# tqch/v-diffusion-torch

Hardware: AMD Instinct MI355X
Metric: train_images_per_sec (higher is better)
Workload: dtype fp32 (bf16x3 split products in the tile-engine GEMMs)

## Files before the change

### v-diffusion-torch_amd/csrc/gemm.hip

```cpp
#include "common.h"
#include <math.h>
#include <stdlib.h>
#include <type_traits>

namespace {

constexpr int KT = 32;
#ifndef VD_GEMM_SPLIT_DEFAULT
#define VD_GEMM_SPLIT_DEFAULT 1
#endif

struct GemmArgs {
    const float* A; const float* B; float* C; const float* bias; const float* R;
    int M, N, K;
    long long lda, ldb, ldc, ldr;
    int nh;
    long long sAb, sAh, sBb, sBh, sCb, sCh, sRb, sRh;
    float alpha; int accumulate;
    int H, W, Cin;
    int kt_total, kt_per_split;
    long long slab_stride;
    float* colsum; int colsum_accumulate;
    int probe;
    float* stats; int stats_hw;
// ... 283 lines not shown
                o[0] = st1; o[p.N] = st2;
            }
        }
    }
}


typedef __attribute__((address_space(3))) void* lds_ptr_t;
constexpr unsigned OOB = 0x80000000u;
#ifndef VD_SCHED_INTERLEAVE
#define VD_SCHED_INTERLEAVE 1
#endif

__device__ __forceinline__ __amdgpu_buffer_rsrc_t make_rsrc(const float* base, int records = (int)OOB) {
    return __builtin_amdgcn_make_buffer_rsrc((void*)base, 0, records, 0x00020000);
}


__device__ __forceinline__ void pix_yx(const GemmArgs& p, int pix, int& y, int& x) {
    if (p.lgW >= 0) { const int rem = pix & ((1 << p.lgHW) - 1); y = rem >> p.lgW; x = rem & ((1 << p.lgW) - 1); }
    else { const int rem = pix % (p.H * p.W); y = rem / p.W; x = rem % p.W; }
}
template <int KT>
__device__ __forceinline__ int swz_of(int row) { return KT == 32 ? ((row >> 1) & 7) : ((row >> 2) & 3); }
template <int KT>
__device__ __forceinline__ int row_swz_t(int row, int chunk) { return row * KT + ((chunk ^ swz_of<KT>(row)) << 2); }

constexpr int VD_GROUP_MAX = 36;
struct GroupPtrs { const float* A[VD_GROUP_MAX]; const float* B[VD_GROUP_MAX]; };
struct NoGroup {};
struct GroupOut { float* C[VD_GROUP_MAX]; float* cs[VD_GROUP_MAX]; };

typedef __bf16 bf16x8 __attribute__((ext_vector_type(8)));
typedef __bf16 bf16x2 __attribute__((ext_vector_type(2)));
__device__ __forceinline__ unsigned pk_bf16(float a, float b) {
    const bf16x2 v = {(__bf16)a, (__bf16)b};
    return __builtin_bit_cast(unsigned, v);
}
__device__ __forceinline__ void split8(const float (&x)[8], bf16x8& H, bf16x8& M, bf16x8& L) {
    typedef unsigned u32x4 __attribute__((ext_vector_type(4)));
    u32x4 h, m, l;
#pragma unroll
    for (int q = 0; q < 4; ++q) {
        const float x0 = x[2 * q], x1 = x[2 * q + 1];
        const unsigned hp = pk_bf16(x0, x1);
        const float r0 = x0 - __uint_as_float(hp << 16), r1 = x1 - __uint_as_float(hp & 0xFFFF0000u);
        const unsigned mp = pk_bf16(r0, r1);
        const float s0 = r0 - __uint_as_float(mp << 16), s1 = r1 - __uint_as_float(mp & 0xFFFF0000u);
        h[q] = hp; m[q] = mp; l[q] = pk_bf16(s0, s1);
    }
    H = __builtin_bit_cast(bf16x8, h); M = __builtin_bit_cast(bf16x8, m); L = __builtin_bit_cast(bf16x8, l);
}

#ifndef VD_KT16_BLOCKS
#define VD_KT16_BLOCKS 4
#endif
#ifndef VD_SPL_BLOCKS
#define VD_SPL_BLOCKS 2
#endif
template <int BM, int BN, int AK, int BK, bool SPLITK, int KT, bool TR, bool GROUPED, bool SPL>
__device__ __forceinline__ void gemm_dma_body(const GemmArgs& p, const std::conditional_t<GROUPED, GroupPtrs, NoGroup>& gp) {
    constexpr int NBUF = 2;
    __shared__ __attribute__((aligned(1024))) float smem[NBUF * (BM + BN) * KT];
    constexpr int MT = BM / 64, NT = BN / 64;
    constexpr int AIT = BM * KT / 1024, BIT = BN * KT / 1024;
    constexpr int A_LPR = BM / 4, B_LPR = BN / 4;
    constexpr int A_RPP = 64 / A_LPR, B_RPP = 64 / B_LPR;
    constexpr int RLPR = KT / 4, RRPP = 64 / RLPR;
    constexpr bool A2 = (AK == VD_COL) && (MT == 2);
    constexpr bool B2 = (BK != VD_ROW) && (NT == 2);
    typedef float f32x2 __attribute__((ext_vector_type(2)));

    const int tid = threadIdx.x, lane = tid & 63;
    const int wave = __builtin_amdgcn_readfirstlane(tid >> 6);
    const int li = lane & 31, lh = lane >> 5;
    const int wm = (wave >> 1) * (BM / 2), wn = (wave & 1) * (BN / 2);
    int tbx = blockIdx.x, tby = blockIdx.y, tbz = blockIdx.z;
    {
        const unsigned T = gridDim.x * gridDim.y * gridDim.z;
        const unsigned lin = (blockIdx.z * gridDim.y + blockIdx.y) * gridDim.x + blockIdx.x;
        if (T >= 16) {
            const unsigned q = T / 8, r = T % 8, xcd = lin % 8, slot = lin / 8;
            const unsigned t = (xcd < r ? xcd * (q + 1) : r * (q + 1) + (xcd - r) * q) + slot;
            tbx = t % gridDim.x; tby = (t / gridDim.x) % gridDim.y; tbz = t / (gridDim.x * gridDim.y);
        }
    }
    const int m0 = tby * BM;
    int n0 = tbx * BN;
    int tapN = 0, ci0 = 0;
    if (BK == VD_IM2COL) {
        const int cchN = (p.Cin + BN - 1) / BN;
        tapN = tbx / cchN;
        ci0 = (tbx % cchN) * BN;
        n0 = tapN * p.Cin + ci0;
    }
    const float* A = p.A;
    const float* B = p.B;
    float* C = p.C;
    const float* R = p.R;
    const float* biasp = p.bias;
    int kt_begin = 0, kt_end = p.kt_total;
    if (SPLITK) {
        int slab = tbz;
        if constexpr (GROUPED) {
            const int e = tbz / p.group_S;
            slab = tbz - e * p.group_S;
            A = gp.A[e];
            B = gp.B[e];
        }
        kt_begin = slab * p.kt_per_split;
        kt_end = min(kt_begin + p.kt_per_split, p.kt_total);
        C += (long long)tbz * p.slab_stride;
    } else {
        const int zb = tbz / p.nh, zh = tbz % p.nh;
        A += zb * p.sAb + zh * p.sAh;
        B += zb * p.sBb + zh * p.sBh;
        C += zb * p.sCb + zh * p.sCh;
        if (R) R += zb * p.sRb + zh * p.sRh;
        if (biasp) biasp += zb * p.sBias;
    }

    unsigned voA[AIT], voB[BIT];
    unsigned mkA[AIT];
    int kcA[AIT], kcB[BIT];
    int by[BIT], bx[BIT];
    int tapA = (AK == VD_IM2COL) ? kt_begin % 9 : 0, ccA = (AK == VD_IM2COL) ? kt_begin / 9 : 0;
    const int kinc_x = (BK == VD_IM2COL) ? KT % p.W : 0, kinc_y = (BK == VD_IM2COL) ? KT / p.W : 0;
#pragma unroll
    for (int j = 0; j < AIT; ++j) {
        const int q = j * 4 + wave;
        if (AK == VD_COL) {
            const int kk = q * A_RPP + lane / A_LPR, cm = (lane % A_LPR) * 4;
            const int rowoff = (GROUPED && p.a_kblk) ? (kk >> 4) * (int)p.a_kblk + (kk & 15) * (int)p.lda : kk * (int)p.lda;
            voA[j] = (m0 + cm < p.M) ? (unsigned)(rowoff + cm) * 4u : OOB;
            kcA[j] = kk; mkA[j] = 0;
        } else {
            const int row = q * RRPP + lane / RLPR;
            const int c = (lane % RLPR) ^ swz_of<KT>(row);
            const int m = m0 + row;
// ... 433 lines not shown
                    if (R) t = __builtin_bit_cast(float, __builtin_amdgcn_raw_buffer_load_b32(rrs, (int)vor, rs * ldr4, 0));
                    if (p.accumulate) t += __builtin_bit_cast(float, __builtin_amdgcn_raw_buffer_load_b32(crs, (int)voc, rs * ldc4, 0));
                }
                addv[r] = t;
            }
#pragma unroll
            for (int r = 0; r < 16; r += 2) {
                const int rs0 = A2 ? 2 * ((r & 3) + 8 * (r >> 2)) + a : 32 * a + (r & 3) + 8 * (r >> 2);
                const int rs1 = A2 ? rs0 + 2 : rs0 + 1;
                f32x2 v = {acc[a][b][r], acc[a][b][r + 1]};
                if (!SPLITK) {
                    const f32x2 al = {p.alpha, p.alpha}, bb = {bv, bv}, ad = {addv[r], addv[r + 1]};
                    v = (v * al + bb) + ad;
                    if (want_stats) {
                        if (!edge) { st1p += v; st2p += v * v; }
                        else {
                            if (rs0 + row_lane < rows_valid) { st1 += v[0]; st2 += v[0] * v[0]; }
                            if (rs1 + row_lane < rows_valid) { st1 += v[1]; st2 += v[1] * v[1]; }
                        }
                    }
                }
                const float v0 = v[0], v1 = v[1];
                __builtin_amdgcn_raw_buffer_store_b32(__float_as_uint(v0), crs, (int)voc, rs0 * ldc4, 0);
                __builtin_amdgcn_raw_buffer_store_b32(__float_as_uint(v1), crs, (int)voc, rs1 * ldc4, 0);
            }
        }
        st1 += st1p[0] + st1p[1];
        st2 += st2p[0] + st2p[1];
        if (want_stats && nok) {
            st1 += __shfl_xor(st1, 32, 64);
            st2 += __shfl_xor(st2, 32, 64);
            const int mrow = m0 + wm;
            if (lh == 0 && mrow < p.M) {
                const int chunks = p.stats_hw / (BM / 2);
                float* o = p.stats + ((long long)(mrow / p.stats_hw) * chunks + (mrow % p.stats_hw) / (BM / 2)) * 2 * p.N + n;
                o[0] = st1; o[p.N] = st2;
            }
        }
    }
    stamp_end();
}

template <int BM, int BN, int AK, int BK, bool SPLITK, int KT, bool TR, bool GROUPED = false>
__global__ __launch_bounds__(256, (KT == 16 ? VD_KT16_BLOCKS : 2)) void gemm_dma_kernel(const GemmArgs p,
                                                                                          const std::conditional_t<GROUPED, GroupPtrs, NoGroup> gp) {
    gemm_dma_body<BM, BN, AK, BK, SPLITK, KT, TR, GROUPED, false>(p, gp);
}
template <int BM, int BN, int AK, int BK, bool SPLITK, int KT, bool TR, bool GROUPED = false>
__global__ __launch_bounds__(256, (KT == 16 ? VD_SPL_BLOCKS : 2)) void gemm_split_kernel(const GemmArgs p,
                                                                                           const std::conditional_t<GROUPED, GroupPtrs, NoGroup> gp) {
    gemm_dma_body<BM, BN, AK, BK, SPLITK, KT, TR, GROUPED, true>(p, gp);
}

__global__ __launch_bounds__(512) void wgrad_planes256_kernel(const GemmArgs p, const GroupPtrs gp) {
    constexpr int BM = 256, BN = 256, KTT = 16, NBUF = 3, STG = (BM + BN) * KTT;
    __shared__ __attribute__((aligned(1024))) float smem[NBUF * STG];
    typedef float f32x2 __attribute__((ext_vector_type(2)));
    const int tid = threadIdx.x, lane = tid & 63;
    const int wave = __builtin_amdgcn_readfirstlane(tid >> 6);
    const int li = lane & 31, lh = lane >> 5;
    const int wm = (wave >> 1) * 64, wn = (wave & 1) * 128;
    const int tbx = blockIdx.x, tby = blockIdx.y, tbz = blockIdx.z;
    const int m0 = tby * BM, n0 = tbx * BN;
    const int e = tbz / p.group_S, slab = tbz - e * p.group_S;
    const float* A = gp.A[e] + m0;
    const float* B = gp.B[e] + n0;
    const int kt_begin = slab * p.kt_per_split, kt_end = min(kt_begin + p.kt_per_split, p.kt_total);
    float* C = p.C + (long long)tbz * p.slab_stride;

    auto issue = [&](int kt, int buf) {
        float* as = smem + buf * STG;
        float* bs = as + BM * KTT;
        const int rec = kt < kt_end ? (int)OOB : 0;
        const __amdgpu_buffer_rsrc_t rsA = make_rsrc(A + (p.a_kblk ? (long long)kt * p.a_kblk : (long long)kt * KTT * p.lda), rec);
        const __amdgpu_buffer_rsrc_t rsB = make_rsrc(B + (p.b_kblk ? (long long)kt * p.b_kblk : (long long)kt * KTT * p.ldb), rec);
#pragma unroll
        for (int h = 0; h < 2; ++h) {
            const int kk = wave + 8 * h;
            __builtin_amdgcn_raw_ptr_buffer_load_lds(rsA, (lds_ptr_t)(as + kk * BM), 16, lane * 16, kk * (int)p.lda * 4, 0, 0);
            __builtin_amdgcn_raw_ptr_buffer_load_lds(rsB, (lds_ptr_t)(bs + kk * BN), 16, lane * 16, kk * (int)p.ldb * 4, 0, 0);
        }
    };

    f32x16 acc[2][4];
#pragma unroll
    for (int a = 0; a < 2; ++a)
#pragma unroll
        for (int b = 0; b < 4; ++b)
#pragma unroll
            for (int r = 0; r < 16; ++r) acc[a][b][r] = 0.f;
    float csum[2] = {0.f, 0.f};
    const bool do_cs = p.colsum != nullptr && tbx == 0 && (wave & 1) == 0;

    if (kt_begin < kt_end) {
        issue(kt_begin, 0);
        issue(kt_begin + 1, 1);
        asm volatile("s_waitcnt vmcnt(4)" ::: "memory");
        asm volatile("s_waitcnt lgkmcnt(0)\n\ts_barrier" ::: "memory");
        int buf = 0;
        for (int kt = kt_begin; kt < kt_end; ++kt) {
            const float* as = smem + buf * STG;
            const float* bs = as + BM * KTT;
            issue(kt + 2, buf >= 1 ? buf - 1 : 2);
            float fa[2][8];
            f32x4 fbq[8];
#pragma unroll
            for (int j = 0; j < 8; ++j) {
                const f32x2 v = *reinterpret_cast<const f32x2*>(as + (8 * lh + j) * BM + wm + 2 * li);
                fa[0][j] = v[0]; fa[1][j] = v[1];
                fbq[j] = *reinterpret_cast<const f32x4*>(bs + (8 * lh + j) * BN + wn + 4 * li);
            }
            bf16x8 ah[2], am[2], al[2];
#pragma unroll
            for (int a = 0; a < 2; ++a) split8(fa[a], ah[a], am[a], al[a]);
            if (do_cs) {
                asm volatile("" ::: "memory");
#pragma unroll
                for (int a = 0; a < 2; ++a)
                    csum[a] += ((fa[a][0] + fa[a][1]) + (fa[a][2] + fa[a][3])) + ((fa[a][4] + fa[a][5]) + (fa[a][6] + fa[a][7]));
            }
#pragma unroll
            for (int hb = 0; hb < 2; ++hb) {
                bf16x8 bh[2], bm[2], bl[2];
#pragma unroll
                for (int b2 = 0; b2 < 2; ++b2) {
                    float fb[8];
#pragma unroll
                    for (int j = 0; j < 8; ++j) fb[j] = fbq[j][2 * hb + b2];
                    split8(fb, bh[b2], bm[b2], bl[b2]);
                }
#pragma unroll
                for (int a = 0; a < 2; ++a)
#pragma unroll
                    for (int b2 = 0; b2 < 2; ++b2) {
                        f32x16& d = acc[a][2 * hb + b2];
                        d = __builtin_amdgcn_mfma_f32_32x32x16_bf16(bl[b2], ah[a], d, 0, 0, 0);
                        d = __builtin_amdgcn_mfma_f32_32x32x16_bf16(bh[b2], al[a], d, 0, 0, 0);
                        d = __builtin_amdgcn_mfma_f32_32x32x16_bf16(bm[b2], am[a], d, 0, 0, 0);
                        d = __builtin_amdgcn_mfma_f32_32x32x16_bf16(bh[b2], am[a], d, 0, 0, 0);
                        d = __builtin_amdgcn_mfma_f32_32x32x16_bf16(bm[b2], ah[a], d, 0, 0, 0);
                        d = __builtin_amdgcn_mfma_f32_32x32x16_bf16(bh[b2], ah[a], d, 0, 0, 0);
                    }
            }
            asm volatile("s_waitcnt vmcnt(4)" ::: "memory");
            asm volatile("s_waitcnt lgkmcnt(0)\n\ts_barrier" ::: "memory");
            buf = buf == 2 ? 0 : buf + 1;
        }
    }
    asm volatile("s_waitcnt vmcnt(0)" ::: "memory");

    if (do_cs) {
#pragma unroll
        for (int a = 0; a < 2; ++a) {
            const float v = csum[a] + __shfl_xor(csum[a], 32, 64);
            if (lh == 0) p.colsum[(long long)tbz * p.M + m0 + wm + 2 * li + a] = v;
        }
    }
    typedef unsigned u32x4 __attribute__((ext_vector_type(4)));
    const __amdgpu_buffer_rsrc_t crs = make_rsrc(C + (long long)m0 * p.N + n0);
#pragma unroll
    for (int a = 0; a < 2; ++a) {
        const unsigned rowb = (unsigned)(wm + 2 * li + a) * (unsigned)p.N * 4u;
#pragma unroll
        for (int r = 0; r < 16; ++r) {
            const int i = (r & 3) + 8 * (r >> 2) + 4 * lh;
            const u32x4 u = {__float_as_uint(acc[a][0][r]), __float_as_uint(acc[a][1][r]), __float_as_uint(acc[a][2][r]), __float_as_uint(acc[a][3][r])};
            __builtin_amdgcn_raw_buffer_store_b128(u, crs, (int)(rowb + (unsigned)(wn + 4 * i) * 4u), 0, 0);
        }
    }
}

__global__ void reduce_slabs_kernel(const float* slabs, int S, long long slab_stride, int M, int N, float* out,
                                    long long ldo, int accumulate, float alpha, const float* cpart, float* colsum,
                                    int colsum_accumulate) {
    const long long idx = (long long)blockIdx.x * blockDim.x + threadIdx.x;
    if (colsum && idx < M) {
        float c = 0.f;
        for (int z = 0; z < S; ++z) c += cpart[(long long)z * M + idx];
        colsum[idx] = colsum_accumulate ? colsum[idx] + c : c;
    }
    if (idx >= (long long)M * N) return;
    float s = 0.f;
    for (int z = 0; z < S; ++z) s += slabs[z * slab_stride + idx];
    const int m = idx / N, n = idx % N;
    float* o = out + (long long)m * ldo + n;
    s *= alpha;
    *o = accumulate ? *o + s : s;
}

__global__ void reduce_slabs_grouped_kernel(const float* slabs, int S, long long slab_stride, int M, int N, const GroupOut outs,
                                            long long ldo, const float* cpart) {
    const int e = blockIdx.y;
    const long long idx = (long long)blockIdx.x * blockDim.x + threadIdx.x;
    const float* sl = slabs + (long long)e * S * slab_stride;
    float* cs = outs.cs[e];
    if (cs && idx < M) {
        float c = 0.f;
        for (int z = 0; z < S; ++z) c += cpart[((long long)e * S + z) * M + idx];
        cs[idx] = c;
    }
    if (idx >= (long long)M * N) return;
    float s = 0.f;
    for (int z = 0; z < S; ++z) s += sl[z * slab_stride + idx];
    const int m = idx / N, n = idx % N;
    outs.C[e][(long long)m * ldo + n] = s;
}

__global__ void reduce_slabs_oihw_kernel(const float* slabs, int S, long long slab_stride, int Cout, int Cin,
                                         int Cout_w, int Cin_w, float* dw, int accumulate, const float* cpart, float* dbias) {
    const long long idx = (long long)blockIdx.x * blockDim.x + threadIdx.x;
    if (dbias && idx < Cout_w) {
        float c = 0.f;
        for (int z = 0; z < S; ++z) c += cpart[(long long)z * Cout + idx];
        dbias[idx] = accumulate ? dbias[idx] + c : c;
    }
    const long long total = (long long)Cout * 9 * Cin;
    if (idx >= total) return;
    const int co = idx / (9 * Cin), rem = idx % (9 * Cin);
    const int tap = rem / Cin, ci = rem % Cin;
    if (co >= Cout_w || ci >= Cin_w) return;
    float s = 0.f;
    for (int z = 0; z < S; ++z) s += slabs[z * slab_stride + idx];
// ... 16 lines not shown
        if (idx < tot) {
            const int ci = idx / (9 * Cout_p), rem = idx % (9 * Cout_p);
            const int tap = rem / Cout_p, co = rem % Cout_p;
            wd[idx] = (co < Cout_w) ? w[((long long)co * Cin_w + ci) * 9 + (8 - tap)] : 0.f;
        }
    }
}


__global__ void pack_conv3x3_batched_kernel(const long long* items, int n) {
    int lo = 0, hi = n - 1;
    while (lo < hi) {
        const int mid = (lo + hi + 1) >> 1;
        if (items[8 * mid + 7] <= (long long)blockIdx.x) lo = mid; else hi = mid - 1;
    }
    const long long* it = items + 8 * lo;
    const float* w = reinterpret_cast<const float*>(it[0]);
    float* wf = reinterpret_cast<float*>(it[1]);
    float* wd = reinterpret_cast<float*>(it[2]);
    const int Cout_w = (int)it[3], Cin_w = (int)it[4], Cin_p = (int)it[5], Cout_p = (int)it[6];
    const long long idx = ((long long)blockIdx.x - it[7]) * blockDim.x + threadIdx.x;
    if (wf) {
        const long long tot = (long long)Cout_w * 9 * Cin_p;
        if (idx < tot) {
            const int co = idx / (9 * Cin_p), rem = idx % (9 * Cin_p);
            const int tap = rem / Cin_p, ci = rem % Cin_p;
            wf[idx] = (ci < Cin_w) ? w[((long long)co * Cin_w + ci) * 9 + tap] : 0.f;
        }
    }
    if (wd) {
        const long long tot = (long long)Cin_w * 9 * Cout_p;
        if (idx < tot) {
            const int ci = idx / (9 * Cout_p), rem = idx % (9 * Cout_p);
            const int tap = rem / Cout_p, co = rem % Cout_p;
            wd[idx] = (co < Cout_w) ? w[((long long)co * Cin_w + ci) * 9 + (8 - tap)] : 0.f;
        }
    }
}


bool dma_in_range(const GemmArgs& a) {
    const long long lim = 0x70000000LL / 4;
    return 128LL * a.lda + 128 < lim && 128LL * a.ldb + 128 < lim && 128LL * a.ldc + 128 < lim && 128LL * a.ldr + 128 < lim &&
           vd_aligned16(a.A) && vd_aligned16(a.B);
}
bool use_dma(const GemmArgs& a) {
    static const bool legacy = getenv("VD_GEMM_LEGACY") != nullptr;
    return !legacy && dma_in_range(a);
}

struct TileCfg { int bm, bn; double eff; int per_cu; };
const TileCfg TILES[4] = {{128, 128, 1.00, 2}, {128, 64, 0.92, 3}, {64, 128, 0.92, 3}, {64, 64, 0.80, 5}};

int choose_tile(long long M, long long Ncols, bool wgrad, long long zcount, int forced) {
    static const char* env = getenv("VD_GEMM_TILE");
    if (env && forced == 0) forced = atoi(env);
    if (forced == 128) return 0;
    if (forced == 12864) return 1;
    if (forced == 64128) return 2;
    if (forced == 64) return 3;
    int best = 0;
    double best_cost = 1e300;
    for (int t = 0; t < 4; ++t) {
        const long long nm = (M + TILES[t].bm - 1) / TILES[t].bm, nn = (Ncols + TILES[t].bn - 1) / TILES[t].bn;
        const double blocks = (double)nm * nn * (wgrad ? 9 : 1) * zcount;
        double cost = (double)(nm * TILES[t].bm) * (double)(nn * TILES[t].bn) / TILES[t].eff;
        if (blocks < 512.0) cost *= sqrt(512.0 / blocks);
        if (cost < best_cost) { best_cost = cost; best = t; }
    }
    return best;
}

inline int ktile_for(const GemmArgs& a, int t, long long nblocks, bool splitk, bool wide, bool wgrad_unsplit = false) {
    static const char* force = getenv("VD_GEMM_KT");
    if (t != 0 || !use_dma(a)) return KT;
    if (wgrad_unsplit) return KT;
    if (force) return atoi(force) == 16 ? 16 : 32;
    if (splitk) return wide ? 16 : 32;
    return nblocks >= 1024 ? 16 : 32;
}

#ifndef VD_WGRAD_WIDE
#define VD_WGRAD_WIDE 32768
#endif
constexpr long long WGRAD_WIDE_PIXELS = VD_WGRAD_WIDE;

bool use_tr(const GemmArgs& a, bool wgrad) {
    static const char* env = getenv("VD_GEMM_TR");
    if (env && atoi(env) == 0) return false;
    if (a.stats && !(a.probe & 32)) return false;
    const long long ncols = wgrad ? a.Cin : a.N;
    if (ncols % 4 || a.ldc % 4 || !vd_aligned16(a.C)) return false;
    if (a.R && (a.ldr % 4 || !vd_aligned16(a.R) || a.sRb % 4 || a.sRh % 4)) return false;
    if (a.bias && (!vd_aligned16(a.bias) || a.sBias % 4)) return false;
    return a.sCb % 4 == 0 && a.sCh % 4 == 0 && a.slab_stride % 4 == 0;
}

static bool split_forms() {
    static const int v = [] { const char* e = getenv("VD_GEMM_SPLIT"); return e ? atoi(e) : VD_GEMM_SPLIT_DEFAULT; }();
    return v != 0;
}
}
extern "C" int vd_gemm_split_forms(void) { return split_forms() ? 1 : 0; }
namespace {
template <bool SPL, int BM, int BN, int AK, int BK, bool SPLITK, int KTV, bool TR, bool GROUPED, class GP>
void launch_dma(const GemmArgs& a, const GP& gp, dim3 grid, hipStream_t st) {
    if constexpr (SPL) hipLaunchKernelGGL((gemm_split_kernel<BM, BN, AK, BK, SPLITK, KTV, TR, GROUPED>), grid, dim3(256), 0, st, a, gp);
    else hipLaunchKernelGGL((gemm_dma_kernel<BM, BN, AK, BK, SPLITK, KTV, TR, GROUPED>), grid, dim3(256), 0, st, a, gp);
}
template <bool SPL, int BM, int BN, int AK, int BK, bool SPLITK, int KT16>
void launch_k16_tr(const GemmArgs& a, dim3 grid, hipStream_t st, bool k16, bool tr) {
    if (k16 && tr) launch_dma<SPL, BM, BN, AK, BK, SPLITK, KT16, true, false>(a, NoGroup{}, grid, st);
    else if (k16) launch_dma<SPL, BM, BN, AK, BK, SPLITK, KT16, false, false>(a, NoGroup{}, grid, st);
    else if (tr) launch_dma<SPL, BM, BN, AK, BK, SPLITK, 32, true, false>(a, NoGroup{}, grid, st);
    else launch_dma<SPL, BM, BN, AK, BK, SPLITK, 32, false, false>(a, NoGroup{}, grid, st);
}

template <int BM, int BN, int AK, int BK, bool SPLITK>
void launch(const GemmArgs& a, dim3 grid, hipStream_t st, int ktile) {
    constexpr bool has16 = BM == 128 && BN == 128 && !(BK == VD_IM2COL && !SPLITK);
    const bool k16 = has16 && ktile == 16;
    const bool tr = use_dma(a) && use_tr(a, BK == VD_IM2COL);
    constexpr bool has_spl = BM == 128 && AK != VD_IM2COL && BK != VD_IM2COL;
    const bool spl = has_spl && use_dma(a) && split_forms();
    vd_g_last_tile = vd_tile_code(tr, spl, use_dma(a) ? (k16 ? 16 : 32) : 0, BM, BN);
    if constexpr (has_spl) {
        if (spl) return launch_k16_tr<true, BM, BN, AK, BK, SPLITK, (has16 ? 16 : 32)>(a, grid, st, k16, tr);
    }
    if (!use_dma(a)) hipLaunchKernelGGL((gemm_kernel<BM, BN, AK, BK, SPLITK>), grid, dim3(256), 0, st, a);
    else launch_k16_tr<false, BM, BN, AK, BK, SPLITK, (has16 ? 16 : 32)>(a, grid, st, k16, tr);
}

template <int AK, int BK, bool SPLITK>
void launch_tile2(int t, const GemmArgs& a, dim3 grid, hipStream_t st, int ktile) {
    if (t == 0) launch<128, 128, AK, BK, SPLITK>(a, grid, st, ktile);
    else if (t == 1) launch<128, 64, AK, BK, SPLITK>(a, grid, st, ktile);
    else if (t == 2) launch<64, 128, AK, BK, SPLITK>(a, grid, st, ktile);
    else launch<64, 64, AK, BK, SPLITK>(a, grid, st, ktile);
}

template <int AK, int BK>
void launch_tile(int t, bool splitk, const GemmArgs& a, dim3 grid, hipStream_t st, int ktile) {
    if (splitk) launch_tile2<AK, BK, true>(t, a, grid, st, ktile);
    else launch_tile2<AK, BK, false>(t, a, grid, st, ktile);
}

int run_gemm(const vd_gemm_desc& d, hipStream_t st) {
    VD_REQUIRE(d.M > 0 && d.N > 0 && d.K > 0, "vd_gemm: empty problem M=%d N=%d K=%d", d.M, d.N, d.K);
    VD_REQUIRE(d.A && d.B && d.C, "vd_gemm: null operand");
    VD_REQUIRE(vd_aligned16(d.A) && vd_aligned16(d.B), "vd_gemm: A/B must be 16-byte aligned");
    VD_REQUIRE(d.lda % 4 == 0 && d.ldb % 4 == 0, "vd_gemm: lda/ldb must be multiples of 4 floats (lda=%lld ldb=%lld)",
               (long long)d.lda, (long long)d.ldb);
    const int ak = d.a_kind, bk = d.b_kind;
    const bool conv = (ak == VD_IM2COL), wgrad = (bk == VD_IM2COL);
    VD_REQUIRE(!(conv && bk != VD_ROW), "vd_gemm: IM2COL A needs ROW B");
    VD_REQUIRE(!(wgrad && ak != VD_COL), "vd_gemm: IM2COL B needs COL A");
    if (ak == VD_ROW) VD_REQUIRE(d.K % 4 == 0, "vd_gemm: K %% 4 != 0 for k-contiguous A (K=%d)", d.K);
    if (ak == VD_COL) VD_REQUIRE(d.M % 4 == 0, "vd_gemm: M %% 4 != 0 for m-contiguous A (M=%d)", d.M);
    if (bk == VD_COL) VD_REQUIRE(d.N % 4 == 0, "vd_gemm: N %% 4 != 0 for n-contiguous B (N=%d)", d.N);
    if (conv || wgrad) VD_REQUIRE(d.Cin % 4 == 0 && d.H > 0 && d.W > 0, "vd_gemm: bad image geometry");
    const int batch = d.batch > 0 ? d.batch : 1;
    const int splitk = d.splitk > 1 ? d.splitk : 1;
    VD_REQUIRE(!(splitk > 1 && batch > 1), "vd_gemm: split-K and batch are exclusive");
    VD_REQUIRE(!(splitk > 1 && (d.bias || d.R)), "vd_gemm: split-K does not take bias/residual");

    GemmArgs a;
    a.A = d.A; a.B = d.B; a.C = d.C; a.bias = d.bias; a.R = d.R;
    a.M = d.M; a.N = d.N; a.K = d.K;
    a.lda = d.lda; a.ldb = d.ldb; a.ldc = d.ldc; a.ldr = d.ldr;
    a.nh = d.nh > 0 ? d.nh : 1;
    a.sAb = d.sAb; a.sAh = d.sAh; a.sBb = d.sBb; a.sBh = d.sBh; a.sCb = d.sCb; a.sCh = d.sCh; a.sRb = d.sRb; a.sRh = d.sRh;
    a.alpha = d.alpha; a.accumulate = d.accumulate;
    a.H = d.H; a.W = d.W; a.Cin = d.Cin;
    a.kt_total = 0; a.kt_per_split = 0; a.slab_stride = 0;
    a.colsum = d.colsum; a.colsum_accumulate = d.colsum_accumulate;
    a.stats = d.stats; a.stats_hw = d.stats_hw;
    a.sBias = d.sBias;
    a.lgW = a.lgHW = -1;
    if ((conv || wgrad) && (d.W & (d.W - 1)) == 0 && ((d.H * d.W) & (d.H * d.W - 1)) == 0) {
        a.lgW = __builtin_ctz((unsigned)d.W); a.lgHW = __builtin_ctz((unsigned)(d.H * d.W));
    }
    a.probe = 0;
#ifdef VD_PROBES
    { static const char* e = getenv("VD_GEMM_PROBE"); a.probe = e ? atoi(e) : 0; }
#endif
    VD_REQUIRE((a.probe & 16) || !(d.colsum && (ak != VD_COL || batch > 1)), "vd_gemm: colsum needs a COL-kind A operand and batch 1");

    const int tile = choose_tile(d.M, wgrad ? d.Cin : d.N, wgrad, (long long)batch * splitk, d.tile);
    const int tbm = TILES[tile].bm, tbn = TILES[tile].bn;
    const long long nm = (d.M + tbm - 1) / tbm;
    const long long nn = wgrad ? 9LL * ((d.Cin + tbn - 1) / tbn) : (d.N + tbn - 1) / tbn;
    VD_REQUIRE(nm <= 65535, "vd_gemm: too many row tiles (%lld)", nm);
    if (d.stats && !(a.probe & 32)) {
        VD_REQUIRE(batch == 1 && splitk == 1 && !wgrad && bk == VD_ROW && ak != VD_COL, "vd_gemm: output statistics need a plain forward launch");
        VD_REQUIRE(d.stats_hw > 0 && d.stats_hw % (tbm / 2) == 0 && d.M % d.stats_hw == 0,
                   "vd_gemm: output statistics need H*W (%d) to be a multiple of half the row tile (%d)", d.stats_hw, tbm / 2);
    }
    const int ktile = ktile_for(a, tile, nm * nn * batch, splitk > 1, wgrad && (long long)d.K >= WGRAD_WIDE_PIXELS, wgrad && splitk <= 1);
    a.kt_total = conv ? 9 * ((d.Cin + ktile - 1) / ktile) : (d.K + ktile - 1) / ktile;
    a.kt_per_split = a.kt_total;

    float* final_C = d.C;
    if (splitk > 1) {
        a.kt_per_split = (a.kt_total + splitk - 1) / splitk;
        const int used = (a.kt_total + a.kt_per_split - 1) / a.kt_per_split;
        a.slab_stride = (long long)d.M * d.N;
        VD_REQUIRE(d.ws && d.ws_bytes >= (int64_t)((used * a.slab_stride + (d.colsum ? (long long)used * d.M : 0)) * 4),
                   "vd_gemm: split-K workspace too small");
        a.C = d.ws; a.ldc = d.N;
        float* cpart = d.ws + used * a.slab_stride;
        if (d.colsum && !(a.probe & 16)) a.colsum = cpart;
        dim3 grid(nn, nm, used);
        if (ak == VD_COL && bk == VD_COL) launch_tile<VD_COL, VD_COL>(tile, true, a, grid, st, ktile);
        else if (ak == VD_COL && bk == VD_IM2COL) launch_tile<VD_COL, VD_IM2COL>(tile, true, a, grid, st, ktile);
        else if (ak == VD_ROW && bk == VD_ROW) launch_tile<VD_ROW, VD_ROW>(tile, true, a, grid, st, ktile);
        else if (ak == VD_ROW && bk == VD_COL) launch_tile<VD_ROW, VD_COL>(tile, true, a, grid, st, ktile);
        else VD_REQUIRE(false, "vd_gemm: split-K not built for kinds (%d,%d)", ak, bk);
        VD_LAUNCH_CHECK("gemm_kernel(splitk)");
        if (!wgrad && !(a.probe & 16)) {
            const long long tot = (long long)d.M * d.N;
            hipLaunchKernelGGL(reduce_slabs_kernel, dim3((tot + 255) / 256), dim3(256), 0, st, d.ws, used, a.slab_stride,
                               d.M, d.N, final_C, d.ldc, d.accumulate, d.alpha, cpart, d.colsum, d.colsum_accumulate);
            VD_LAUNCH_CHECK("reduce_slabs_kernel");
        }
        return 0;
    }
    dim3 grid(nn, nm, batch);
    if (ak == VD_ROW && bk == VD_ROW) launch_tile<VD_ROW, VD_ROW>(tile, false, a, grid, st, ktile);
    else if (ak == VD_ROW && bk == VD_COL) launch_tile<VD_ROW, VD_COL>(tile, false, a, grid, st, ktile);
    else if (ak == VD_COL && bk == VD_COL) launch_tile<VD_COL, VD_COL>(tile, false, a, grid, st, ktile);
    else if (ak == VD_COL && bk == VD_ROW) launch_tile<VD_COL, VD_ROW>(tile, false, a, grid, st, ktile);
    else if (ak == VD_IM2COL && bk == VD_ROW) launch_tile<VD_IM2COL, VD_ROW>(tile, false, a, grid, st, ktile);
    else if (ak == VD_COL && bk == VD_IM2COL) launch_tile<VD_COL, VD_IM2COL>(tile, false, a, grid, st, ktile);
    else VD_REQUIRE(false, "vd_gemm: unsupported operand kinds (%d,%d)", ak, bk);
    VD_LAUNCH_CHECK("gemm_kernel");
    return 0;
}

template <int BM, int BN, int KTV = 32>
void launch_grouped(const GemmArgs& a, const GroupPtrs& gp, dim3 grid, hipStream_t st) {
    const bool spl = split_forms();
    vd_g_last_tile = vd_tile_code(true, spl, KTV, BM, BN);
    if (spl) launch_dma<true, BM, BN, VD_COL, VD_COL, true, KTV, true, true>(a, gp, grid, st);
    else launch_dma<false, BM, BN, VD_COL, VD_COL, true, KTV, true, true>(a, gp, grid, st);
}
constexpr long long GROUPED_K16_MIN_WGS = 768;
static bool planes256(int count, int M, int N, int K) {
    static const bool on = !(getenv("VD_PLANES256") && atoi(getenv("VD_PLANES256")) == 0);
    if (!(on && split_forms() && M % 256 == 0 && N % 256 == 0 && K % 16 == 0)) return false;
    const long long blocks = (long long)(M / 256) * (N / 256) * count, slots = vd_cu_count();
    const int kmax = K / 256 > 1 ? K / 256 : 1;
    double best = 0.0;
    for (int sl = 1; sl <= 24 && sl <= kmax; ++sl) {
        const long long wgs = blocks * sl, rounds = (wgs + slots - 1) / slots;
        const double eff = (double)wgs / (double)(rounds * slots);
        if (eff > best) best = eff;
    }
    return best >= 0.85;
}

void grouped_tiles(int tile, bool p256, int M, int N, long long* nm, long long* nn) {
    const int bm = p256 ? 256 : TILES[tile].bm, bn = p256 ? 256 : TILES[tile].bn;
    *nm = (M + bm - 1) / bm; *nn = (N + bn - 1) / bn;
}

struct GroupedPlan { int tile; bool p256, k16; long long nm, nn; int kt_total, kt_per_split, used; };
GroupedPlan plan_grouped(int count, int M, int N, int K, int S) {
    GroupedPlan g;
    g.tile = choose_tile(M, N, false, (long long)count * S, 0);
    g.p256 = planes256(count, M, N, K);
    grouped_tiles(g.tile, g.p256, M, N, &g.nm, &g.nn);
    g.k16 = g.p256 || (g.tile == 0 && g.nm * g.nn * count * S >= GROUPED_K16_MIN_WGS);
    g.kt_total = g.k16 ? (K + 15) / 16 : (K + 31) / 32;
    g.kt_per_split = (g.kt_total + S - 1) / S;
    g.used = (g.kt_total + g.kt_per_split - 1) / g.kt_per_split;
    return g;
}
}

extern "C" int vd_gemm_grouped_wgrad_auto_split(int32_t count, int32_t M, int32_t N, int32_t K, int32_t min_slabs, int32_t max_slabs) {
    const int tile = choose_tile(M, N, false, (long long)count * 8, 0);
    const bool p256 = planes256(count, M, N, K);
    long long nm, nn;
    grouped_tiles(tile, p256, M, N, &nm, &nn);
    const long long blocks = nm * nn * count;
    const long long slots = (long long)vd_cu_count() * (p256 ? 1 : (tile == 0 && blocks * (min_slabs > 1 ? min_slabs : 1) >= GROUPED_K16_MIN_WGS / 2 ? 4 : TILES[tile].per_cu));
    int lo = min_slabs > 1 ? min_slabs : 1, hi = max_slabs > lo ? max_slabs : lo;
    const int kmax = K / 256 > 1 ? K / 256 : 1;
    if (hi > kmax) hi = kmax;
    if (lo > hi) lo = hi;
    int best = lo;
    double best_eff = -1.0;
    for (int s = lo; s <= hi; ++s) {
        const long long wgs = blocks * s, rounds = (wgs + slots - 1) / slots;
        double eff = (double)wgs / (double)(rounds * slots);
        eff *= 1.0 - 0.004 * s;
        if (eff > best_eff) { best_eff = eff; best = s; }
    }
    return best;
}

extern "C" size_t vd_gemm_grouped_wgrad_ws_bytes(int32_t count, int32_t M, int32_t N, int32_t splitk) {
// ... 192 lines not shown
```

### v-diffusion-torch_amd/v_diffusion/_hip.py

```python
import ctypes as C
import os

import torch

_HERE = os.path.dirname(os.path.abspath(__file__))
LIB_PATH = os.environ.get("VDIFF_HIP_LIB") or os.path.join(os.path.dirname(_HERE), "lib", "libvdiff_hip.so")

ROW, COL, IM2COL = 0, 1, 2
RS_NONE, RS_DOWN, RS_UP = 0, 1, 2
OUT_TYPES = {"v": 0, "x0": 1, "eps": 2, "both": 3}
REWEIGHTS = {"constant": 0, "snr": 1, "snr_trunc": 2, "snr_1plus": 3}

_i32, _i64, _f32, _f64, _u64, _vp, _sz = C.c_int32, C.c_int64, C.c_float, C.c_double, C.c_uint64, C.c_void_p, C.c_size_t


class GemmDesc(C.Structure):
    _fields_ = [("A", _vp), ("B", _vp), ("C", _vp), ("bias", _vp), ("R", _vp),
                ("M", _i32), ("N", _i32), ("K", _i32), ("a_kind", _i32), ("b_kind", _i32),
                ("lda", _i64), ("ldb", _i64), ("ldc", _i64), ("ldr", _i64),
                ("batch", _i32), ("nh", _i32),
                ("sAb", _i64), ("sAh", _i64), ("sBb", _i64), ("sBh", _i64),
                ("sCb", _i64), ("sCh", _i64), ("sRb", _i64), ("sRh", _i64),
                ("alpha", _f32), ("accumulate", _i32), ("H", _i32), ("W", _i32), ("Cin", _i32),
                ("splitk", _i32), ("ws", _vp), ("ws_bytes", _i64), ("tile", _i32),
# ... 145 lines not shown
    if not t.is_cuda:
        raise HipError("v_diffusion HIP op received a CPU tensor: the hot path runs on an MI355X only (no CPU fallback)")
    if t.dtype not in (torch.float32, torch.float64, torch.uint8, torch.int32):
        raise HipError(f"unsupported dtype {t.dtype}")
    return t.data_ptr()


def stream():
    return torch.cuda.current_stream().cuda_stream


_ws_cache = {}

PROFILE = None
PROFILE_BYTES = {}
_KIND = {0: "ROW", 1: "COL", 2: "IM2COL"}


def _note_bytes(name, nbytes):
    if PROFILE is not None:
        e = PROFILE_BYTES.setdefault(name, [0.0, 0])
        e[0] += float(nbytes)
        e[1] += 1


def tile_fields(code):
    flags = code // 100000000
    return bool(flags & 1), flags >= 2, (code // 1000000) % 100, (code // 1000) % 1000, code % 1000


class _Timed:
    def __init__(self, name, amount, rename=None):
        self.name, self.amount, self.rename = name, amount, rename

    def __enter__(self):
        if PROFILE is not None:
            self.e0, self.e1 = torch.cuda.Event(enable_timing=True), torch.cuda.Event(enable_timing=True)
            self.e0.record()
        return self

    def __exit__(self, *exc):
        if PROFILE is not None and exc[0] is None:
            self.e1.record()
            PROFILE.append(self._record() + (self.e0, self.e1))


class _TimedTile(_Timed):
    def _record(self):
        tr, spl, kt, bm, bn = tile_fields(lib().vd_gemm_last_tile())
        name = self.name.format(tile=f"{bm}, {bn}", kt=f"{kt}, {'true' if tr else 'false'}")
        if spl:
            name = name.replace("gemm_dma_kernel", "gemm_split_kernel")
        if spl and (bm, bn) == (256, 256):
            name = "wgrad_planes256_kernel" + name[name.index(">") + 1:]
        if kt == 0:
            name = name.replace("gemm_dma_kernel", "gemm_kernel").replace(", 0, false>", ">")
        return name, self.amount


class _TimedName(_Timed):
    def _record(self):
        return self.name, self.amount


class _TimedBytes(_Timed):
    def _record(self):
        return "hbm:" + (self.rename() if self.rename else self.name), float(self.amount)


def _two_parts(parts):
    (p1, c1, k1), (p2, c2, k2) = parts[0], (parts[1] if len(parts) > 1 else (None, 0, 0))
    return ptr(p1), c1, k1, ptr(p2), c2, k2


def _resampled(H, W, resample):
    return (H // 2, W // 2) if resample == RS_DOWN else ((H * 2, W * 2) if resample == RS_UP else (H, W))


def _resampled_hw(H, W, resample):
    Ho, Wo = _resampled(H, W, resample)
    return Ho * Wo


def _wgrad_args(x, ldx, dy, lddy, nimg, H, W, Cin, Cout, dw, dbias, Cin_w, Cout_w, accumulate, ws):
    return (ptr(x), ldx, ptr(dy), lddy, nimg, H, W, Cin, Cout, ptr(dw), ptr(dbias), Cin_w, Cout_w, int(accumulate), ws.data_ptr(),
            ws.numel() * 4)


def workspace(nbytes, device, tag="default"):
    key = (device, torch.cuda.current_stream(device).cuda_stream, tag)
    buf = _ws_cache.get(key)
    if buf is None or buf.numel() * 4 < nbytes:
        buf = torch.empty((max(int(nbytes), 1 << 20) + 3) // 4, dtype=torch.float32, device=device)
        _ws_cache[key] = buf
    return buf


def gemm(A, B, Cm, M, N, K, *, a_kind=ROW, b_kind=ROW, lda, ldb, ldc, bias=None, R=None, ldr=0, batch=1, nh=1,
         sA=(0, 0), sB=(0, 0), sC=(0, 0), sR=(0, 0), alpha=1.0, accumulate=False, splitk=1, tile=0, colsum=None,
         colsum_accumulate=False, stats=None, stats_hw=0, sBias=0):
    d = GemmDesc()
    d.A, d.B, d.C, d.bias, d.R = ptr(A), ptr(B), ptr(Cm), ptr(bias), ptr(R)
    d.M, d.N, d.K, d.a_kind, d.b_kind = M, N, K, a_kind, b_kind
    d.lda, d.ldb, d.ldc, d.ldr = lda, ldb, ldc, ldr
    d.batch, d.nh = batch, nh
    (d.sAb, d.sAh), (d.sBb, d.sBh), (d.sCb, d.sCh), (d.sRb, d.sRh) = sA, sB, sC, sR
    d.alpha, d.accumulate = alpha, int(accumulate)
# ... 566 lines not shown
```

Before: 2165.

## Generalize 256x256 planes kernel to ungrouped GEMMs with fused epilogue

Turns the grouped wgrad 256x256 split-bf16 kernel into a template over operand layouts (row or column) and adds an ungrouped variant with alpha, bias, residual and accumulate applied in the epilogue plus XCD-aware tile ordering. Large row-row GEMMs (M of at least 131072, K of at least 512) are routed to it by default to get more data reuse per workgroup and fewer tile loads. In exchange, occupancy drops to one 512-thread block with a large LDS footprint, and the new swizzled row-major DMA path adds risk.

```diff
diff --git a/v-diffusion-torch_amd/csrc/gemm.hip b/v-diffusion-torch_amd/csrc/gemm.hip
--- a/v-diffusion-torch_amd/csrc/gemm.hip
+++ b/v-diffusion-torch_amd/csrc/gemm.hip
@@ -359,6 +359,17 @@
     H = __builtin_bit_cast(bf16x8, h); M = __builtin_bit_cast(bf16x8, m); L = __builtin_bit_cast(bf16x8, l);
 }
 
+__device__ __forceinline__ void xcd_tile_order(int& tbx, int& tby, int& tbz) {
+    tbx = blockIdx.x; tby = blockIdx.y; tbz = blockIdx.z;
+    const unsigned T = gridDim.x * gridDim.y * gridDim.z;
+    const unsigned lin = (blockIdx.z * gridDim.y + blockIdx.y) * gridDim.x + blockIdx.x;
+    if (T >= 16) {
+        const unsigned q = T / 8, r = T % 8, xcd = lin % 8, slot = lin / 8;
+        const unsigned t = (xcd < r ? xcd * (q + 1) : r * (q + 1) + (xcd - r) * q) + slot;
+        tbx = t % gridDim.x; tby = (t / gridDim.x) % gridDim.y; tbz = t / (gridDim.x * gridDim.y);
+    }
+}
+
 #ifndef VD_KT16_BLOCKS
 #define VD_KT16_BLOCKS 4
 #endif
@@ -382,16 +393,8 @@
     const int wave = __builtin_amdgcn_readfirstlane(tid >> 6);
     const int li = lane & 31, lh = lane >> 5;
     const int wm = (wave >> 1) * (BM / 2), wn = (wave & 1) * (BN / 2);
-    int tbx = blockIdx.x, tby = blockIdx.y, tbz = blockIdx.z;
-    {
-        const unsigned T = gridDim.x * gridDim.y * gridDim.z;
-        const unsigned lin = (blockIdx.z * gridDim.y + blockIdx.y) * gridDim.x + blockIdx.x;
-        if (T >= 16) {
-            const unsigned q = T / 8, r = T % 8, xcd = lin % 8, slot = lin / 8;
-            const unsigned t = (xcd < r ? xcd * (q + 1) : r * (q + 1) + (xcd - r) * q) + slot;
-            tbx = t % gridDim.x; tby = (t / gridDim.x) % gridDim.y; tbz = t / (gridDim.x * gridDim.y);
-        }
-    }
+    int tbx, tby, tbz;
+    xcd_tile_order(tbx, tby, tbz);
     const int m0 = tby * BM;
     int n0 = tbx * BN;
     int tapN = 0, ci0 = 0;
@@ -931,33 +934,112 @@
     gemm_dma_body<BM, BN, AK, BK, SPLITK, KT, TR, GROUPED, true>(p, gp);
 }
 
-__global__ __launch_bounds__(512) void wgrad_planes256_kernel(const GemmArgs p, const GroupPtrs gp) {
-    constexpr int BM = 256, BN = 256, KTT = 16, NBUF = 3, STG = (BM + BN) * KTT;
+namespace p256 {
+constexpr int BM = 256, BN = 256, KTT = 16, NBUF = 3, WAVES = 8, STG = (BM + BN) * KTT;
+constexpr int PIECES = BM * KTT / 256 / WAVES;
+constexpr int DMA_PER_TILE = 2 * PIECES;
+static_assert(BM == BN && PIECES * WAVES * 256 == BM * KTT && NBUF == 3, "one piece plan for both operands; the loop below is written for three stages");
+
+template <int KIND, int NB>
+__device__ __forceinline__ int own_row(int b, int i) { return KIND == VD_COL ? NB * i + b : 32 * b + i; }
+
+template <int KIND>
+__device__ __forceinline__ void dma_piece(__amdgpu_buffer_rsrc_t rs, float* tile, int h, unsigned vo, int ld, int wave, int lane) {
+    const int q = wave + WAVES * h;
+    if (KIND == VD_COL) __builtin_amdgcn_raw_ptr_buffer_load_lds(rs, (lds_ptr_t)(tile + q * BM), 16, lane * 16, q * ld * 4, 0, 0);
+    else __builtin_amdgcn_raw_ptr_buffer_load_lds(rs, (lds_ptr_t)(tile + q * 256), 16, (int)vo, 0, 0, 0);
+}
+template <int KIND>
+__device__ __forceinline__ unsigned piece_offset(int h, int ld, int wave, int lane) {
+    if (KIND == VD_COL) return 0u;
+    const int row = (wave + WAVES * h) * 16 + (lane >> 2);
+    return (unsigned)(row * ld + (((lane & 3) ^ swz_of<KTT>(row)) << 2)) * 4u;
+}
+
+template <int KIND, int NB>
+__device__ __forceinline__ void load_frags(const float* tile, int w0, int li, int lh, float (&f)[NB][8]) {
+    if (KIND == VD_COL) {
+        typedef float vec __attribute__((ext_vector_type(NB)));
+#pragma unroll
+        for (int j = 0; j < 8; ++j) {
+            const vec v = *reinterpret_cast<const vec*>(tile + (8 * lh + j) * BM + w0 + NB * li);
+#pragma unroll
+            for (int b = 0; b < NB; ++b) f[b][j] = v[b];
+        }
+    } else {
+#pragma unroll
+        for (int b = 0; b < NB; ++b) {
+            const int row = w0 + 32 * b + li;
+            const f32x4 q0 = *reinterpret_cast<const f32x4*>(tile + row_swz_t<KTT>(row, 2 * lh));
+            const f32x4 q1 = *reinterpret_cast<const f32x4*>(tile + row_swz_t<KTT>(row, 2 * lh + 1));
+#pragma unroll
+            for (int j = 0; j < 4; ++j) { f[b][j] = q0[j]; f[b][4 + j] = q1[j]; }
+        }
+    }
+}
+
+template <bool XL_FIRST>
+__device__ __forceinline__ void mfma6(f32x16& d, bf16x8 xh, bf16x8 xm, bf16x8 xl, bf16x8 yh, bf16x8 ym, bf16x8 yl) {
+    if (XL_FIRST) {
+        d = __builtin_amdgcn_mfma_f32_32x32x16_bf16(xl, yh, d, 0, 0, 0);
+        d = __builtin_amdgcn_mfma_f32_32x32x16_bf16(xh, yl, d, 0, 0, 0);
+    } else {
+        d = __builtin_amdgcn_mfma_f32_32x32x16_bf16(xh, yl, d, 0, 0, 0);
+        d = __builtin_amdgcn_mfma_f32_32x32x16_bf16(xl, yh, d, 0, 0, 0);
+    }
+    d = __builtin_amdgcn_mfma_f32_32x32x16_bf16(xm, ym, d, 0, 0, 0);
+    d = __builtin_amdgcn_mfma_f32_32x32x16_bf16(xh, ym, d, 0, 0, 0);
+    d = __builtin_amdgcn_mfma_f32_32x32x16_bf16(xm, yh, d, 0, 0, 0);
+    d = __builtin_amdgcn_mfma_f32_32x32x16_bf16(xh, yh, d, 0, 0, 0);
+}
+}
+
+template <int AK, int BK, bool GROUPED>
+__device__ __forceinline__ void planes256_body(const GemmArgs& p, const std::conditional_t<GROUPED, GroupPtrs, NoGroup>& gp) {
+    using namespace p256;
     __shared__ __attribute__((aligned(1024))) float smem[NBUF * STG];
-    typedef float f32x2 __attribute__((ext_vector_type(2)));
     const int tid = threadIdx.x, lane = tid & 63;
     const int wave = __builtin_amdgcn_readfirstlane(tid >> 6);
     const int li = lane & 31, lh = lane >> 5;
     const int wm = (wave >> 1) * 64, wn = (wave & 1) * 128;
-    const int tbx = blockIdx.x, tby = blockIdx.y, tbz = blockIdx.z;
+    int tbx = blockIdx.x, tby = blockIdx.y, tbz = blockIdx.z;
+    if constexpr (!GROUPED) xcd_tile_order(tbx, tby, tbz);
     const int m0 = tby * BM, n0 = tbx * BN;
-    const int e = tbz / p.group_S, slab = tbz - e * p.group_S;
-    const float* A = gp.A[e] + m0;
-    const float* B = gp.B[e] + n0;
-    const int kt_begin = slab * p.kt_per_split, kt_end = min(kt_begin + p.kt_per_split, p.kt_total);
-    float* C = p.C + (long long)tbz * p.slab_stride;
+    const float* A = p.A;
+    const float* B = p.B;
+    float* C = p.C;
+    int kt_begin = 0, kt_end = p.kt_total;
+    long long a_kblk = 0, b_kblk = 0;
+    if constexpr (GROUPED) {
+        const int e = tbz / p.group_S, slab = tbz - e * p.group_S;
+        A = gp.A[e];
+        B = gp.B[e];
+        kt_begin = slab * p.kt_per_split;
+        kt_end = min(kt_begin + p.kt_per_split, p.kt_total);
+        C += (long long)tbz * p.slab_stride;
+        a_kblk = p.a_kblk; b_kblk = p.b_kblk;
+    }
+    A += (AK == VD_COL) ? (long long)m0 : (long long)m0 * p.lda;
+    B += (BK == VD_COL) ? (long long)n0 : (long long)n0 * p.ldb;
+    unsigned voA[PIECES], voB[PIECES];
+#pragma unroll
+    for (int h = 0; h < PIECES; ++h) {
+        voA[h] = piece_offset<AK>(h, (int)p.lda, wave, lane);
+        voB[h] = piece_offset<BK>(h, (int)p.ldb, wave, lane);
+    }
 
     auto issue = [&](int kt, int buf) {
         float* as = smem + buf * STG;
         float* bs = as + BM * KTT;
         const int rec = kt < kt_end ? (int)OOB : 0;
-        const __amdgpu_buffer_rsrc_t rsA = make_rsrc(A + (p.a_kblk ? (long long)kt * p.a_kblk : (long long)kt * KTT * p.lda), rec);
-        const __amdgpu_buffer_rsrc_t rsB = make_rsrc(B + (p.b_kblk ? (long long)kt * p.b_kblk : (long long)kt * KTT * p.ldb), rec);
-#pragma unroll
-        for (int h = 0; h < 2; ++h) {
-            const int kk = wave + 8 * h;
-            __builtin_amdgcn_raw_ptr_buffer_load_lds(rsA, (lds_ptr_t)(as + kk * BM), 16, lane * 16, kk * (int)p.lda * 4, 0, 0);
-            __builtin_amdgcn_raw_ptr_buffer_load_lds(rsB, (lds_ptr_t)(bs + kk * BN), 16, lane * 16, kk * (int)p.ldb * 4, 0, 0);
+        const long long ka = AK == VD_COL ? (a_kblk ? (long long)kt * a_kblk : (long long)kt * KTT * p.lda) : (long long)kt * KTT;
+        const long long kb = BK == VD_COL ? (b_kblk ? (long long)kt * b_kblk : (long long)kt * KTT * p.ldb) : (long long)kt * KTT;
+        const __amdgpu_buffer_rsrc_t rsA = make_rsrc(A + ka, rec);
+        const __amdgpu_buffer_rsrc_t rsB = make_rsrc(B + kb, rec);
+#pragma unroll
+        for (int h = 0; h < PIECES; ++h) {
+            dma_piece<AK>(rsA, as, h, voA[h], (int)p.lda, wave, lane);
+            dma_piece<BK>(rsB, bs, h, voB[h], (int)p.ldb, wave, lane);
         }
     };
 
@@ -969,30 +1051,25 @@
 #pragma unroll
             for (int r = 0; r < 16; ++r) acc[a][b][r] = 0.f;
     float csum[2] = {0.f, 0.f};
-    const bool do_cs = p.colsum != nullptr && tbx == 0 && (wave & 1) == 0;
+    const bool do_cs = GROUPED && p.colsum != nullptr && tbx == 0 && (wave & 1) == 0;
 
     if (kt_begin < kt_end) {
         issue(kt_begin, 0);
         issue(kt_begin + 1, 1);
-        asm volatile("s_waitcnt vmcnt(4)" ::: "memory");
+        asm volatile("s_waitcnt vmcnt(%0)" ::"n"(DMA_PER_TILE) : "memory");
         asm volatile("s_waitcnt lgkmcnt(0)\n\ts_barrier" ::: "memory");
         int buf = 0;
         for (int kt = kt_begin; kt < kt_end; ++kt) {
             const float* as = smem + buf * STG;
             const float* bs = as + BM * KTT;
             issue(kt + 2, buf >= 1 ? buf - 1 : 2);
-            float fa[2][8];
-            f32x4 fbq[8];
-#pragma unroll
-            for (int j = 0; j < 8; ++j) {
-                const f32x2 v = *reinterpret_cast<const f32x2*>(as + (8 * lh + j) * BM + wm + 2 * li);
-                fa[0][j] = v[0]; fa[1][j] = v[1];
-                fbq[j] = *reinterpret_cast<const f32x4*>(bs + (8 * lh + j) * BN + wn + 4 * li);
-            }
+            float fa[2][8], fb[4][8];
+            load_frags<AK, 2>(as, wm, li, lh, fa);
+            load_frags<BK, 4>(bs, wn, li, lh, fb);
             bf16x8 ah[2], am[2], al[2];
 #pragma unroll
             for (int a = 0; a < 2; ++a) split8(fa[a], ah[a], am[a], al[a]);
-            if (do_cs) {
+            if (GROUPED && do_cs) {
                 asm volatile("" ::: "memory");
 #pragma unroll
                 for (int a = 0; a < 2; ++a)
@@ -1002,51 +1079,74 @@
             for (int hb = 0; hb < 2; ++hb) {
                 bf16x8 bh[2], bm[2], bl[2];
 #pragma unroll
-                for (int b2 = 0; b2 < 2; ++b2) {
-                    float fb[8];
-#pragma unroll
-                    for (int j = 0; j < 8; ++j) fb[j] = fbq[j][2 * hb + b2];
-                    split8(fb, bh[b2], bm[b2], bl[b2]);
-                }
+                for (int b2 = 0; b2 < 2; ++b2) split8(fb[2 * hb + b2], bh[b2], bm[b2], bl[b2]);
 #pragma unroll
                 for (int a = 0; a < 2; ++a)
 #pragma unroll
-                    for (int b2 = 0; b2 < 2; ++b2) {
-                        f32x16& d = acc[a][2 * hb + b2];
-                        d = __builtin_amdgcn_mfma_f32_32x32x16_bf16(bl[b2], ah[a], d, 0, 0, 0);
-                        d = __builtin_amdgcn_mfma_f32_32x32x16_bf16(bh[b2], al[a], d, 0, 0, 0);
-                        d = __builtin_amdgcn_mfma_f32_32x32x16_bf16(bm[b2], am[a], d, 0, 0, 0);
-                        d = __builtin_amdgcn_mfma_f32_32x32x16_bf16(bh[b2], am[a], d, 0, 0, 0);
-                        d = __builtin_amdgcn_mfma_f32_32x32x16_bf16(bm[b2], ah[a], d, 0, 0, 0);
-                        d = __builtin_amdgcn_mfma_f32_32x32x16_bf16(bh[b2], ah[a], d, 0, 0, 0);
-                    }
-            }
-            asm volatile("s_waitcnt vmcnt(4)" ::: "memory");
+                    for (int b2 = 0; b2 < 2; ++b2)
+                        mfma6<GROUPED>(acc[a][2 * hb + b2], bh[b2], bm[b2], bl[b2], ah[a], am[a], al[a]);
+            }
+            asm volatile("s_waitcnt vmcnt(%0)" ::"n"(DMA_PER_TILE) : "memory");
             asm volatile("s_waitcnt lgkmcnt(0)\n\ts_barrier" ::: "memory");
             buf = buf == 2 ? 0 : buf + 1;
         }
     }
     asm volatile("s_waitcnt vmcnt(0)" ::: "memory");
 
-    if (do_cs) {
+    if (GROUPED && do_cs) {
 #pragma unroll
         for (int a = 0; a < 2; ++a) {
             const float v = csum[a] + __shfl_xor(csum[a], 32, 64);
-            if (lh == 0) p.colsum[(long long)tbz * p.M + m0 + wm + 2 * li + a] = v;
+            if (lh == 0) p.colsum[(long long)tbz * p.M + m0 + wm + own_row<AK, 2>(a, li)] = v;
         }
     }
     typedef unsigned u32x4 __attribute__((ext_vector_type(4)));
-    const __amdgpu_buffer_rsrc_t crs = make_rsrc(C + (long long)m0 * p.N + n0);
+    const int ldc4 = (int)p.ldc * 4, ldr4 = (int)p.ldr * 4;
+    const float* R = GROUPED ? nullptr : p.R;
+    const float* biasp = GROUPED ? nullptr : p.bias;
+    const __amdgpu_buffer_rsrc_t crs = make_rsrc(C + (long long)m0 * p.ldc + n0);
+    const __amdgpu_buffer_rsrc_t rrs = make_rsrc(R ? R + (long long)m0 * p.ldr + n0 : C, R ? (int)OOB : 0);
+    const f32x4 al4 = {p.alpha, p.alpha, p.alpha, p.alpha};
 #pragma unroll
     for (int a = 0; a < 2; ++a) {
-        const unsigned rowb = (unsigned)(wm + 2 * li + a) * (unsigned)p.N * 4u;
-#pragma unroll
-        for (int r = 0; r < 16; ++r) {
-            const int i = (r & 3) + 8 * (r >> 2) + 4 * lh;
-            const u32x4 u = {__float_as_uint(acc[a][0][r]), __float_as_uint(acc[a][1][r]), __float_as_uint(acc[a][2][r]), __float_as_uint(acc[a][3][r])};
-            __builtin_amdgcn_raw_buffer_store_b128(u, crs, (int)(rowb + (unsigned)(wn + 4 * i) * 4u), 0, 0);
-        }
-    }
+        const int rowl = wm + own_row<AK, 2>(a, li);
+#pragma unroll
+        for (int e0 = 0; e0 < 16; e0 += 4) {
+            f32x4 bias4[4], add4[4];
+            unsigned vocs[4];
+#pragma unroll
+            for (int ee = 0; ee < 4; ++ee) {
+                const int e = e0 + ee;
+                const int ncol = wn + (BK == VD_COL ? 4 * ((e & 3) + 8 * (e >> 2) + 4 * lh) : 32 * (e >> 2) + 8 * (e & 3) + 4 * lh);
+                vocs[ee] = (unsigned)(rowl * ldc4 + ncol * 4);
+                if constexpr (!GROUPED) {
+                    bias4[ee] = biasp ? *reinterpret_cast<const f32x4*>(biasp + n0 + ncol) : f32x4{0.f, 0.f, 0.f, 0.f};
+                    f32x4 t = {0.f, 0.f, 0.f, 0.f};
+                    if (R) t = __builtin_bit_cast(f32x4, __builtin_amdgcn_raw_buffer_load_b128(rrs, (int)(rowl * ldr4 + ncol * 4), 0, 0));
+                    if (p.accumulate) t += __builtin_bit_cast(f32x4, __builtin_amdgcn_raw_buffer_load_b128(crs, (int)vocs[ee], 0, 0));
+                    add4[ee] = t;
+                }
+            }
+#pragma unroll
+            for (int ee = 0; ee < 4; ++ee) {
+                const int e = e0 + ee;
+                f32x4 v;
+                if (BK == VD_COL) v = f32x4{acc[a][0][e], acc[a][1][e], acc[a][2][e], acc[a][3][e]};
+                else v = f32x4{acc[a][e >> 2][4 * (e & 3)], acc[a][e >> 2][4 * (e & 3) + 1], acc[a][e >> 2][4 * (e & 3) + 2], acc[a][e >> 2][4 * (e & 3) + 3]};
+                if constexpr (!GROUPED) v = (v * al4 + bias4[ee]) + add4[ee];
+                const u32x4 u = {__float_as_uint(v[0]), __float_as_uint(v[1]), __float_as_uint(v[2]), __float_as_uint(v[3])};
+                __builtin_amdgcn_raw_buffer_store_b128(u, crs, (int)vocs[ee], 0, 0);
+            }
+        }
+    }
+}
+
+__global__ __launch_bounds__(512) void wgrad_planes256_kernel(const GemmArgs p, const GroupPtrs gp) {
+    planes256_body<VD_COL, VD_COL, true>(p, gp);
+}
+template <int AK, int BK>
+__global__ __launch_bounds__(512) void gemm_planes256_kernel(const GemmArgs p) {
+    planes256_body<AK, BK, false>(p, NoGroup{});
 }
 
 __global__ void reduce_slabs_kernel(const float* slabs, int S, long long slab_stride, int M, int N, float* out,
@@ -1169,9 +1269,12 @@
 struct TileCfg { int bm, bn; double eff; int per_cu; };
 const TileCfg TILES[4] = {{128, 128, 1.00, 2}, {128, 64, 0.92, 3}, {64, 128, 0.92, 3}, {64, 64, 0.80, 5}};
 
+int forced_tile(int forced) {
+    static const char* env = getenv("VD_GEMM_TILE");
+    return (env && forced == 0) ? atoi(env) : forced;
+}
 int choose_tile(long long M, long long Ncols, bool wgrad, long long zcount, int forced) {
-    static const char* env = getenv("VD_GEMM_TILE");
-    if (env && forced == 0) forced = atoi(env);
+    forced = forced_tile(forced);
     if (forced == 128) return 0;
     if (forced == 12864) return 1;
     if (forced == 64128) return 2;
@@ -1217,6 +1320,10 @@
     static const int v = [] { const char* e = getenv("VD_GEMM_SPLIT"); return e ? atoi(e) : VD_GEMM_SPLIT_DEFAULT; }();
     return v != 0;
 }
+static bool planes256_on() {
+    static const bool on = !(getenv("VD_PLANES256") && atoi(getenv("VD_PLANES256")) == 0);
+    return on && split_forms();
+}
 }
 extern "C" int vd_gemm_split_forms(void) { return split_forms() ? 1 : 0; }
 namespace {
@@ -1260,6 +1367,31 @@
 void launch_tile(int t, bool splitk, const GemmArgs& a, dim3 grid, hipStream_t st, int ktile) {
     if (splitk) launch_tile2<AK, BK, true>(t, a, grid, st, ktile);
     else launch_tile2<AK, BK, false>(t, a, grid, st, ktile);
+}
+
+constexpr int GEMM256_MIN_ROWS = 32768, GEMM256_GATE_ROWS = 131072, GEMM256_GATE_K = 512;
+bool plan_gemm256(const vd_gemm_desc& d, const GemmArgs& a, int batch, int splitk) {
+    const int forced = forced_tile(d.tile);
+    if (!planes256_on() || (forced != 0 && forced != 256) || !use_dma(a) || a.probe) return false;
+    if (batch != 1 || splitk != 1 || d.stats || d.colsum) return false;
+    const bool kinds = (d.a_kind == VD_ROW && (d.b_kind == VD_ROW || d.b_kind == VD_COL)) || (d.a_kind == VD_COL && d.b_kind == VD_COL);
+    if (!kinds || d.M % 256 || d.N % 256 || d.K % p256::KTT || d.M < GEMM256_MIN_ROWS) return false;
+    const bool gate = d.a_kind == VD_ROW && d.b_kind == VD_ROW && d.K >= GEMM256_GATE_K && d.M >= GEMM256_GATE_ROWS;
+    if (forced != 256 && !gate) return false;
+    const long long lim = 0x70000000LL / 4;
+    if (256LL * a.lda + 256 >= lim || 256LL * a.ldb + 256 >= lim || 256LL * a.ldc + 256 >= lim || 256LL * a.ldr + 256 >= lim) return false;
+    return use_tr(a, false);
+}
+int launch_gemm256(const vd_gemm_desc& d, GemmArgs& a, hipStream_t st) {
+    a.kt_total = a.kt_per_split = d.K / p256::KTT;
+    const dim3 grid(d.N / 256, d.M / 256, 1);
+    VD_REQUIRE(grid.y <= 65535, "vd_gemm: too many row tiles (%u)", grid.y);
+    vd_g_last_tile = vd_tile_code(true, true, p256::KTT, 256, 256);
+    if (d.a_kind == VD_ROW && d.b_kind == VD_ROW) hipLaunchKernelGGL((gemm_planes256_kernel<VD_ROW, VD_ROW>), grid, dim3(512), 0, st, a);
+    else if (d.a_kind == VD_ROW) hipLaunchKernelGGL((gemm_planes256_kernel<VD_ROW, VD_COL>), grid, dim3(512), 0, st, a);
+    else hipLaunchKernelGGL((gemm_planes256_kernel<VD_COL, VD_COL>), grid, dim3(512), 0, st, a);
+    VD_LAUNCH_CHECK("gemm_planes256_kernel");
+    return 0;
 }
 
 int run_gemm(const vd_gemm_desc& d, hipStream_t st) {
@@ -1303,6 +1435,7 @@
 #endif
     VD_REQUIRE((a.probe & 16) || !(d.colsum && (ak != VD_COL || batch > 1)), "vd_gemm: colsum needs a COL-kind A operand and batch 1");
 
+    if (plan_gemm256(d, a, batch, splitk)) return launch_gemm256(d, a, st);
     const int tile = choose_tile(d.M, wgrad ? d.Cin : d.N, wgrad, (long long)batch * splitk, d.tile);
     const int tbm = TILES[tile].bm, tbn = TILES[tile].bn;
     const long long nm = (d.M + tbm - 1) / tbm;
@@ -1363,8 +1496,7 @@
 }
 constexpr long long GROUPED_K16_MIN_WGS = 768;
 static bool planes256(int count, int M, int N, int K) {
-    static const bool on = !(getenv("VD_PLANES256") && atoi(getenv("VD_PLANES256")) == 0);
-    if (!(on && split_forms() && M % 256 == 0 && N % 256 == 0 && K % 16 == 0)) return false;
+    if (!(planes256_on() && M % 256 == 0 && N % 256 == 0 && K % 16 == 0)) return false;
     const long long blocks = (long long)(M / 256) * (N / 256) * count, slots = vd_cu_count();
     const int kmax = K / 256 > 1 ? K / 256 : 1;
     double best = 0.0;
diff --git a/v-diffusion-torch_amd/v_diffusion/_hip.py b/v-diffusion-torch_amd/v_diffusion/_hip.py
--- a/v-diffusion-torch_amd/v_diffusion/_hip.py
+++ b/v-diffusion-torch_amd/v_diffusion/_hip.py
@@ -221,7 +221,9 @@
         if spl:
             name = name.replace("gemm_dma_kernel", "gemm_split_kernel")
         if spl and (bm, bn) == (256, 256):
-            name = "wgrad_planes256_kernel" + name[name.index(">") + 1:]
+            kinds = self.name.split(", ")[1:3]
+            grouped = self.name.endswith("true, true>")
+            name = "wgrad_planes256_kernel" if grouped else f"gemm_planes256_kernel<{kinds[0]}, {kinds[1]}>"
         if kt == 0:
             name = name.replace("gemm_dma_kernel", "gemm_kernel").replace(", 0, false>", ">")
         return name, self.amount
```

New measurement: 2148. About the same (-0.8%).
